# flyakon/DeepPhysiNet

Measured on AMD Instinct MI355X. Metric: collocation-points/sec (fwd+PDE-Jacobian+bwd), higher is better.
Workload: dtype bf16x2 (hi+lo split bf16 MFMA operands), fp32 accumulate

## Files before the change

deepphysinet_amd/csrc/dpn_encoder_chain.hip:

```cpp
#include <atomic>
#include <hip/hip_runtime.h>
#include <stdint.h>
#include <stdlib.h>

#include "../../include/dpn_hip.h"
#include "../../include/dpn_hip_experiments.h"

#define DEV __device__ __forceinline__

namespace {

typedef _Float16 f16x8 __attribute__((ext_vector_type(8)));
typedef float f32x4 __attribute__((ext_vector_type(4)));
typedef unsigned int u32;
typedef u32 u32x4 __attribute__((ext_vector_type(4)));

constexpr int kD = 256;
constexpr int kThreads = 512, kWaves = 8;
constexpr int kImgBytes = 256 * 1024;
#ifndef DPN_ENC_PF
#define DPN_ENC_PF 8
#endif
template <int NTT> constexpr int pf_of() { return NTT == 1 ? DPN_ENC_PF : 4; }
constexpr int kYS = 260;
constexpr int kXImg = 16384;
constexpr float kLoScale = 2048.0f, kLoInv = 1.0f / 2048.0f;

#ifdef DPN_ENC_TIMELINE
unsigned* g_enc_timeline = nullptr;
#define ENC_STAMP(I) do { if (a.tl && lane == 0) a.tl[((size_t)blockIdx.x * kWaves + wave) * 32 + (I)] = (unsigned)__builtin_readcyclecounter(); } while (0)
#define ENC_TL_ARG unsigned* tl;
#define ENC_TL_SET(A) (A).tl = g_enc_timeline
#else
#define ENC_STAMP(I) do { } while (0)
#define ENC_TL_ARG
#define ENC_TL_SET(A) do { } while (0)
#endif

DEV void barrier_lds() {
    __builtin_amdgcn_fence(__ATOMIC_RELEASE, "workgroup", "local");
    __builtin_amdgcn_s_barrier();
    __builtin_amdgcn_fence(__ATOMIC_ACQUIRE, "workgroup", "local");
}

template <int CTRL>
DEV float dpp(float v) { return __builtin_bit_cast(float, __builtin_amdgcn_update_dpp(0, __builtin_bit_cast(int, v), CTRL, 0xf, 0xf, false)); }
DEV float swz16(float v) { return __builtin_bit_cast(float, __builtin_amdgcn_ds_swizzle(__builtin_bit_cast(int, v), 0x401F)); }
DEV float half_sum(float v) {
    v += dpp<0xB1>(v);
    v += dpp<0x4E>(v);
    v += dpp<0x141>(v);
    v += dpp<0x140>(v);
    v += swz16(v);
    return v;
}
DEV float half_max(float v) {
    v = fmaxf(v, dpp<0xB1>(v));
    v = fmaxf(v, dpp<0x4E>(v));
    v = fmaxf(v, dpp<0x141>(v));
    v = fmaxf(v, dpp<0x140>(v));
    v = fmaxf(v, swz16(v));
    return v;
}

DEV float gelu_exact(float x) { return x * 0.5f * (1.0f + erff(x * 0.70710678118654752440f)); }
DEV float gelu_exact_grad(float x) {
    const float cdf = 0.5f * (1.0f + erff(x * 0.70710678118654752440f));
    const float pdf = expf(-0.5f * x * x) * 0.39894228040143267794f;
    return cdf + x * pdf;
}

DEV void split8(const float (&v)[8], u32x4& hi, u32x4& lo) {
    f16x8 h, l;
#pragma unroll
    for (int e = 0; e < 8; ++e) {
        const _Float16 a = (_Float16)v[e];
        h[e] = a;
        l[e] = (_Float16)((v[e] - (float)a) * kLoScale);
    }
    hi = __builtin_bit_cast(u32x4, h);
    lo = __builtin_bit_cast(u32x4, l);
}

DEV int xpos(int slot, int n) { return slot * 16 + (n ^ ((slot & 3) | ((slot & 4) ? 12 : 0))); }

struct RowLane {
    int tsel, slot, n16;
    DEV RowLane(int wave, int lane) : tsel(lane >> 5), slot(lane & 31), n16(2 * wave + (lane >> 5)) {}
};

DEV void row_to_ximg(const float (&v)[8], const float extra_max, const RowLane& rl, char* ximg_tile, float* rscale_tile) {
    float m = extra_max;
#pragma unroll
    for (int e = 0; e < 8; ++e) m = fmaxf(m, fabsf(v[e]));
    m = half_max(m);
    int eb = (__builtin_bit_cast(int, m) >> 23) & 0xff;
    eb = eb < 4 ? 4 : eb;
    const float sc = __builtin_bit_cast(float, (257 - eb) << 23);
    float s[8];
#pragma unroll
    for (int e = 0; e < 8; ++e) s[e] = v[e] * sc;
    u32x4 hi, lo;
    split8(s, hi, lo);
    char* p = ximg_tile + xpos(rl.slot, rl.n16) * 16;
    *reinterpret_cast<u32x4*>(p) = hi;
    *reinterpret_cast<u32x4*>(p + kXImg / 2) = lo;
    if (rl.slot == 0) rscale_tile[rl.n16] = __builtin_bit_cast(float, (eb - 3) << 23);
}
DEV float row_absmax(const float (&v)[8]) {
    float m = 0.f;
#pragma unroll
    for (int e = 0; e < 8; ++e) m = fmaxf(m, fabsf(v[e]));
    return m;
}

DEV void load8(float (&v)[8], const float* p, bool ok) {
    if (ok) {
        const float4 a = reinterpret_cast<const float4*>(p)[0], b = reinterpret_cast<const float4*>(p)[1];
        v[0] = a.x; v[1] = a.y; v[2] = a.z; v[3] = a.w; v[4] = b.x; v[5] = b.y; v[6] = b.z; v[7] = b.w;
    } else {
#pragma unroll
        for (int e = 0; e < 8; ++e) v[e] = 0.f;
    }
}
DEV void store8(float* p, const float (&v)[8], bool ok) {
    if (ok) {
        reinterpret_cast<float4*>(p)[0] = make_float4(v[0], v[1], v[2], v[3]);
        reinterpret_cast<float4*>(p)[1] = make_float4(v[4], v[5], v[6], v[7]);
    }
}
DEV void lds8(float (&v)[8], const float* p) {
    const f32x4 a = reinterpret_cast<const f32x4*>(p)[0], b = reinterpret_cast<const f32x4*>(p)[1];
    v[0] = a[0]; v[1] = a[1]; v[2] = a[2]; v[3] = a[3]; v[4] = b[0]; v[5] = b[1]; v[6] = b[2]; v[7] = b[3];
}

DEV void layer_norm8(const float (&v)[8], const float (&gam)[8], const float (&bet)[8], float (&xhat)[8], float (&y)[8], float& rstd) {
    float s = 0.f;
#pragma unroll
    for (int e = 0; e < 8; ++e) s += v[e];
    const float mean = half_sum(s) * (1.f / kD);
    float d[8], q = 0.f;
#pragma unroll
    for (int e = 0; e < 8; ++e) { d[e] = v[e] - mean; q = fmaf(d[e], d[e], q); }
    rstd = 1.0f / sqrtf(half_sum(q) * (1.f / kD) + 1e-5f);
#pragma unroll
    for (int e = 0; e < 8; ++e) { xhat[e] = d[e] * rstd; y[e] = fmaf(xhat[e], gam[e], bet[e]); }
}
DEV void layer_norm_bwd8(const float (&g)[8], const float (&xhat)[8], const float rstd, const float (&gam)[8], float (&gx)[8], float (&pg)[8],
                         float (&pb)[8]) {
    float t[8], s1 = 0.f, s2 = 0.f;
#pragma unroll
    for (int e = 0; e < 8; ++e) { t[e] = g[e] * gam[e]; s1 += t[e]; s2 = fmaf(t[e], xhat[e], s2); pg[e] = fmaf(g[e], xhat[e], pg[e]); pb[e] += g[e]; }
    const float m1 = half_sum(s1) * (1.f / kD), m2 = half_sum(s2) * (1.f / kD);
#pragma unroll
    for (int e = 0; e < 8; ++e) gx[e] = rstd * (t[e] - m1 - xhat[e] * m2);
}

struct WStream {
    __amdgpu_buffer_rsrc_t rs;
    int voff, tile_off;
    DEV void init(const void* wpack, int64_t bytes, int wave, int lane) {
        rs = __builtin_amdgcn_make_buffer_rsrc(const_cast<void*>(wpack), 0, (int)bytes, 0x00020000);
        voff = lane * 16;
        tile_off = wave * 2 * 16384;
    }
    DEV void load(u32x4 (&dst)[2][2], int img_off, int ks) const {
#pragma unroll
        for (int t = 0; t < 2; ++t)
#pragma unroll
            for (int p = 0; p < 2; ++p)
                dst[t][p] = __builtin_bit_cast(u32x4, __builtin_amdgcn_raw_buffer_load_b128(rs, voff + p * 1024, img_off + tile_off + t * 16384 + ks * 2048, 0));
    }
};
template <int PF> struct Ring { u32x4 a[PF][2][2]; };

DEV f32x4 mfma(u32x4 a, u32x4 b, f32x4 c) {
    return __builtin_amdgcn_mfma_f32_16x16x32_f16(__builtin_bit_cast(f16x8, a), __builtin_bit_cast(f16x8, b), c, 0, 0, 0);
}

template <int NTT>
struct Acc {
    f32x4 m[2][NTT], c[2][NTT];
    DEV void zero() {
#pragma unroll
        for (int t = 0; t < 2; ++t)
#pragma unroll
            for (int tt = 0; tt < NTT; ++tt) { m[t][tt] = (f32x4)0.f; c[t][tt] = (f32x4)0.f; }
    }
};

template <int NTT, bool HAS_NEXT>
DEV void gemm(const WStream& ws, Ring<pf_of<NTT>()>& R, const int cur_off, const int next_off, const char* xr0, const char* xr1, Acc<NTT>& acc) {
    u32x4 B[2][NTT][2];
    auto loadB = [&](const int ks, const int buf) __attribute__((always_inline)) {
        const char* base = ((ks & 1) ? xr1 : xr0) + ks * 1024;
#pragma unroll
        for (int tt = 0; tt < NTT; ++tt) {
            B[buf][tt][0] = *reinterpret_cast<const u32x4*>(base + tt * kXImg);
            B[buf][tt][1] = *reinterpret_cast<const u32x4*>(base + tt * kXImg + kXImg / 2);
        }
    };
    constexpr int kPF = pf_of<NTT>();
    loadB(0, 0);
#pragma unroll
    for (int ks = 0; ks < 8; ++ks) {
        if (ks + 1 < 8) loadB(ks + 1, (ks + 1) & 1);
        const int s = ks % kPF, b = ks & 1;
#pragma unroll
        for (int tt = 0; tt < NTT; ++tt) {
#pragma unroll
            for (int t = 0; t < 2; ++t) acc.m[t][tt] = mfma(R.a[s][t][0], B[b][tt][0], acc.m[t][tt]);
#pragma unroll
            for (int t = 0; t < 2; ++t) acc.c[t][tt] = mfma(R.a[s][t][0], B[b][tt][1], acc.c[t][tt]);
#pragma unroll
            for (int t = 0; t < 2; ++t) acc.c[t][tt] = mfma(R.a[s][t][1], B[b][tt][0], acc.c[t][tt]);
        }
        if (ks + kPF < 8) ws.load(R.a[s], cur_off, ks + kPF);
        else if (HAS_NEXT) ws.load(R.a[s], next_off, ks + kPF - 8);
    }
}

template <int NTT>
DEV void acc_to_staging(const Acc<NTT>& acc, float* Y, const float* rscale, int wave, int lane) {
    const int n = lane & 15, g = lane >> 4;
#pragma unroll
    for (int tt = 0; tt < NTT; ++tt) {
        const float rs = rscale[tt * 16 + n];
#pragma unroll
        for (int t = 0; t < 2; ++t) {
            f32x4 v;
#pragma unroll
            for (int j = 0; j < 4; ++j) v[j] = fmaf(acc.c[t][tt][j], kLoInv, acc.m[t][tt][j]) * rs;
            *reinterpret_cast<f32x4*>(Y + (tt * 16 + n) * kYS + wave * 32 + t * 16 + g * 4) = v;
        }
    }
}
template <int NTT>
DEV void acc_to_global(const Acc<NTT>& acc, float* out, const float* bias_lds, const float* rscale, int row0, int rows, int wave, int lane) {
    const int n = lane & 15, g = lane >> 4;
#pragma unroll
    for (int tt = 0; tt < NTT; ++tt) {
        const float rs = rscale[tt * 16 + n];
        const int row = row0 + tt * 16 + n;
#pragma unroll
        for (int t = 0; t < 2; ++t) {
            const int ch = wave * 32 + t * 16 + g * 4;
            f32x4 b = (f32x4)0.f;
            if (bias_lds) b = *reinterpret_cast<const f32x4*>(bias_lds + ch);
            f32x4 v;
#pragma unroll
            for (int j = 0; j < 4; ++j) v[j] = fmaf(acc.c[t][tt][j], kLoInv, acc.m[t][tt][j]) * rs + b[j];
            if (row < rows) *reinterpret_cast<f32x4*>(out + (int64_t)row * kD + ch) = v;
        }
    }
}

constexpr int kHelpers = 64;
DEV void l2_warm_helper(const void* wpack, const int (&img)[6], const int n_img, const int hb) {
    const int part = hb >> 3, t = threadIdx.x;
    float sum = 0.f;
    for (int i = t >> 8; i < n_img; i += 2) {
        const char* p = static_cast<const char*>(wpack) + img[i] + (part * 256 + (t & 255)) * 128;
        sum += *reinterpret_cast<const float*>(p);
    }
    asm volatile("" ::"v"(sum));
}

constexpr int kNVecF = 12;
enum { VF_BO = 0, VF_G1, VF_BE1, VF_BC1, VF_BC2, VF_G2, VF_BE2, VF_GF, VF_BEF, VF_BN0, VF_BN1, VF_BN2 };
struct FwdArgs {
    const void* wpack;
    int64_t wbytes;
    int img[6];
    int rows, n_main, n_img;
    const float *o, *x, *xin;
    const float* vec[kNVecF];
    float *x1, *xhat1, *rstd1, *pre, *act, *x2, *xhat2, *rstd2, *xf, *xhatf, *rstdf, *y0, *y1, *y2;
    const float *emb_parts, *emb_bias, *emb_pos, *emb_te, *emb_token;
    float* emb_out;
    int64_t emb_part_stride;
    int emb_n_parts, emb_n_tok;
    ENC_TL_ARG
};
template <int NTT>
struct Lds {
    static constexpr int kX = 0;
    static constexpr int kY = 3 * NTT * kXImg;
    static constexpr int kVec = kY + NTT * 16 * kYS * 4;
    static constexpr int kRs = kVec + kNVecF * 256 * 4;
    static constexpr int kRed = kRs + NTT * 16 * 4;
    static constexpr int kBytes = kRed + kWaves * 512 * 4;
};

constexpr int kEmbAhead = 9;
template <bool TAIL, int NEXT, int NTT>
__global__ __launch_bounds__(kThreads) void dpn_enc_fwd_kernel(FwdArgs a) {
    extern __shared__ __attribute__((aligned(16))) char smem[];
    char* ximg = smem + Lds<NTT>::kX;
    float* Y = reinterpret_cast<float*>(smem + Lds<NTT>::kY);
    float* vecs = reinterpret_cast<float*>(smem + Lds<NTT>::kVec);
    float* rscale = reinterpret_cast<float*>(smem + Lds<NTT>::kRs);
    const int tid = threadIdx.x, lane = tid & 63, wave = __builtin_amdgcn_readfirstlane(tid >> 6);
    if ((int)blockIdx.x >= a.n_main) { l2_warm_helper(a.wpack, a.img, a.n_img, blockIdx.x - a.n_main); return; }
    const int row0 = blockIdx.x * 16 * NTT;
    ENC_STAMP(0);
    const RowLane rl(wave, lane);
    const int n_r = lane & 15, g_r = lane >> 4;
    const char* xr0 = ximg + (g_r * 16 + (n_r ^ g_r)) * 16;
    const char* xr1 = ximg + (g_r * 16 + (n_r ^ g_r ^ 12)) * 16;
    float res[NTT][8], vin[NTT][8];
    bool ok[NTT];
#pragma unroll
    for (int tt = 0; tt < NTT; ++tt) {
        const int row = row0 + tt * 16 + rl.n16;
        ok[tt] = row < a.rows;
        if constexpr (!TAIL) {
            if (a.emb_parts) {
                const int c0 = rl.slot * 8;
                const bool tok = row < a.emb_n_tok;
                const int64_t po = ((int64_t)(tok ? 0 : row - a.emb_n_tok)) * kD + c0;
                float v[8];
                if (tok) load8(v, a.emb_token + (int64_t)row * kD + c0, ok[tt]);
                else load8(v, a.emb_parts + po, ok[tt]);
                if (!tok)
                    for (int p0 = 1; p0 < a.emb_n_parts; p0 += kEmbAhead) {
                        float t6[kEmbAhead][8];
#pragma unroll
                        for (int u = 0; u < kEmbAhead; ++u) load8(t6[u], a.emb_parts + (int64_t)min(p0 + u, a.emb_n_parts - 1) * a.emb_part_stride + po, ok[tt]);
#pragma unroll
                        for (int u = 0; u < kEmbAhead; ++u)
                            if (p0 + u < a.emb_n_parts) {
#pragma unroll
                                for (int e = 0; e < 8; ++e) v[e] += t6[u][e];
                            }
                    }
                float b8[8], p8[8], e8[8];
                load8(b8, a.emb_bias + c0, !tok && a.emb_bias != nullptr);
                load8(p8, a.emb_pos + (int64_t)row * kD + c0, ok[tt]);
                load8(e8, a.emb_te + c0, true);
#pragma unroll
                for (int e = 0; e < 8; ++e) vin[tt][e] = ok[tt] ? ((tok ? v[e] : v[e] + b8[e]) + p8[e]) + e8[e] : 0.f;
                store8(a.emb_out + (int64_t)row * kD + c0, vin[tt], ok[tt]);
                continue;
            }
        }
        load8(vin[tt], (TAIL ? a.o : a.xin) + (int64_t)row * kD + rl.slot * 8, ok[tt]);
        if constexpr (TAIL) load8(res[tt], a.x + (int64_t)row * kD + rl.slot * 8, ok[tt]);
    }
    constexpr int kVecLoads = (kNVecF * 64 + kThreads - 1) / kThreads;
    float4 pv[kVecLoads];
#pragma unroll
    for (int q = 0; q < kVecLoads; ++q) {
        const int i = tid + q * kThreads;
        const float* src = i < kNVecF * 64 ? a.vec[i >> 6] : nullptr;
        pv[q] = src ? reinterpret_cast<const float4*>(src)[i & 63] : make_float4(0.f, 0.f, 0.f, 0.f);
    }
    WStream ws;
    ws.init(a.wpack, a.wbytes, wave, lane);
    constexpr int kPF = pf_of<NTT>();
    Ring<kPF> R;
#pragma unroll
    for (int ks = 0; ks < kPF; ++ks) ws.load(R.a[ks], a.img[0], ks);
#pragma unroll
    for (int q = 0; q < kVecLoads; ++q) {
        const int i = tid + q * kThreads;
        if (i < kNVecF * 64) reinterpret_cast<float4*>(vecs)[i] = pv[q];
    }
#pragma unroll
    for (int tt = 0; tt < NTT; ++tt) row_to_ximg(vin[tt], 0.f, rl, ximg + tt * kXImg, rscale + tt * 16);
    ENC_STAMP(1);
    barrier_lds();
    ENC_STAMP(2);
    Acc<NTT> acc;
    constexpr int kFirstNext = TAIL ? 3 : 0;
    if constexpr (TAIL) {
        acc.zero();
        gemm<NTT, true>(ws, R, a.img[0], a.img[1], xr0, xr1, acc);
        ENC_STAMP(3);
        acc_to_staging<NTT>(acc, Y, rscale, wave, lane);
        barrier_lds();
        ENC_STAMP(4);
        float sa[NTT][8], sb[NTT][8], sr[NTT];
        {
            float gam[8], bet[8], bo[8];
            lds8(bo, vecs + VF_BO * 256 + rl.slot * 8); lds8(gam, vecs + VF_G1 * 256 + rl.slot * 8); lds8(bet, vecs + VF_BE1 * 256 + rl.slot * 8);
#pragma unroll
            for (int tt = 0; tt < NTT; ++tt) {
                float v[8];
                lds8(v, Y + (tt * 16 + rl.n16) * kYS + rl.slot * 8);
#pragma unroll
                for (int e = 0; e < 8; ++e) v[e] = res[tt][e] + (v[e] + bo[e]);
                layer_norm8(v, gam, bet, sb[tt], res[tt], sr[tt]);
                row_to_ximg(res[tt], 0.f, rl, ximg + tt * kXImg, rscale + tt * 16);
            }
        }
        ENC_STAMP(5);
        barrier_lds();
        ENC_STAMP(6);
#pragma unroll
        for (int tt = 0; tt < NTT; ++tt) {
            const int64_t off = (int64_t)(row0 + tt * 16 + rl.n16) * kD + rl.slot * 8;
            store8(a.x1 + off, res[tt], ok[tt]);
            store8(a.xhat1 + off, sb[tt], ok[tt]);
            if (ok[tt] && rl.slot == 0) a.rstd1[row0 + tt * 16 + rl.n16] = sr[tt];
        }
        acc.zero();
        gemm<NTT, true>(ws, R, a.img[1], a.img[2], xr0, xr1, acc);
        ENC_STAMP(7);
        acc_to_staging<NTT>(acc, Y, rscale, wave, lane);
        barrier_lds();
        ENC_STAMP(8);
        {
            float b1[8];
            lds8(b1, vecs + VF_BC1 * 256 + rl.slot * 8);
#pragma unroll
            for (int tt = 0; tt < NTT; ++tt) {
                lds8(sa[tt], Y + (tt * 16 + rl.n16) * kYS + rl.slot * 8);
#pragma unroll
                for (int e = 0; e < 8; ++e) { sa[tt][e] += b1[e]; sb[tt][e] = gelu_exact(sa[tt][e]); }
                row_to_ximg(sb[tt], 0.f, rl, ximg + tt * kXImg, rscale + tt * 16);
            }
        }
        ENC_STAMP(9);
        barrier_lds();
        ENC_STAMP(10);
#pragma unroll
        for (int tt = 0; tt < NTT; ++tt) {
            const int64_t off = (int64_t)(row0 + tt * 16 + rl.n16) * kD + rl.slot * 8;
            store8(a.pre + off, sa[tt], ok[tt]);
            store8(a.act + off, sb[tt], ok[tt]);
        }
        acc.zero();
        gemm<NTT, NEXT != 0>(ws, R, a.img[2], a.img[3], xr0, xr1, acc);
        ENC_STAMP(11);
        acc_to_staging<NTT>(acc, Y, rscale, wave, lane);
        barrier_lds();
        ENC_STAMP(12);
        float sc[NEXT == 2 ? NTT : 1][8], sd[NEXT == 2 ? NTT : 1][8], sq[NEXT == 2 ? NTT : 1];
        {
            float gam[8], bet[8], b2[8];
            lds8(b2, vecs + VF_BC2 * 256 + rl.slot * 8); lds8(gam, vecs + VF_G2 * 256 + rl.slot * 8); lds8(bet, vecs + VF_BE2 * 256 + rl.slot * 8);
#pragma unroll
            for (int tt = 0; tt < NTT; ++tt) {
                float v[8];
                lds8(v, Y + (tt * 16 + rl.n16) * kYS + rl.slot * 8);
#pragma unroll
                for (int e = 0; e < 8; ++e) v[e] = res[tt][e] + (v[e] + b2[e]);
                layer_norm8(v, gam, bet, sb[tt], sa[tt], sr[tt]);
                if constexpr (NEXT == 2) {
                    float gf[8], bf[8];
                    lds8(gf, vecs + VF_GF * 256 + rl.slot * 8); lds8(bf, vecs + VF_BEF * 256 + rl.slot * 8);
                    layer_norm8(sa[tt], gf, bf, sd[tt], sc[tt], sq[tt]);
                    row_to_ximg(sc[tt], 0.f, rl, ximg + tt * kXImg, rscale + tt * 16);
                } else if constexpr (NEXT == 1) {
                    row_to_ximg(sa[tt], 0.f, rl, ximg + tt * kXImg, rscale + tt * 16);
                }
            }
        }
        ENC_STAMP(13);
        if constexpr (NEXT != 0) barrier_lds();
        ENC_STAMP(14);
#pragma unroll
        for (int tt = 0; tt < NTT; ++tt) {
            const int64_t off = (int64_t)(row0 + tt * 16 + rl.n16) * kD + rl.slot * 8;
            store8(a.x2 + off, sa[tt], ok[tt]);
            store8(a.xhat2 + off, sb[tt], ok[tt]);
            if (ok[tt] && rl.slot == 0) a.rstd2[row0 + tt * 16 + rl.n16] = sr[tt];
            if constexpr (NEXT == 2) {
                store8(a.xf + off, sc[tt], ok[tt]);
                store8(a.xhatf + off, sd[tt], ok[tt]);
                if (ok[tt] && rl.slot == 0) a.rstdf[row0 + tt * 16 + rl.n16] = sq[tt];
            }
        }
    }
    if constexpr (NEXT == 1) {
        acc.zero();
        gemm<NTT, true>(ws, R, a.img[kFirstNext], a.img[kFirstNext + 1], xr0, xr1, acc);
        acc_to_global<NTT>(acc, a.y0, vecs + VF_BN0 * 256, rscale, row0, a.rows, wave, lane);
        ENC_STAMP(15);
        acc.zero();
        gemm<NTT, true>(ws, R, a.img[kFirstNext + 1], a.img[kFirstNext + 2], xr0, xr1, acc);
        acc_to_global<NTT>(acc, a.y1, vecs + VF_BN1 * 256, rscale, row0, a.rows, wave, lane);
        ENC_STAMP(16);
        acc.zero();
        gemm<NTT, false>(ws, R, a.img[kFirstNext + 2], 0, xr0, xr1, acc);
        acc_to_global<NTT>(acc, a.y2, vecs + VF_BN2 * 256, rscale, row0, a.rows, wave, lane);
        ENC_STAMP(17);
    } else if constexpr (NEXT == 2) {
        acc.zero();
        gemm<NTT, false>(ws, R, a.img[kFirstNext], 0, xr0, xr1, acc);
        acc_to_global<NTT>(acc, a.y0, vecs + VF_BN0 * 256, rscale, row0, a.rows, wave, lane);
    }
}

enum { VB_G2 = 0, VB_G1, VB_GF };
struct BwdArgs {
    const void* wpack;
    int64_t wbytes;
    int img[6];
    int rows, n_main, n_img;
    const float *res, *dq, *dk, *dv;
    const float *dmeta, *xhatf, *rstdf;
    const float* gin;
    const float *xhat2, *rstd2, *pre, *xhat1, *rstd1;
    const float* vec[3];
    float *gs2, *dpre, *gs1, *dout, *gx;
    float *partial_f, *partial2, *partial1;
    float* gx_head;
    int gx_head_rows;
    ENC_TL_ARG
};

DEV void partials_to_lds(float (&pg)[8], float (&pb)[8], float* red, int wave, int lane) {
#pragma unroll
    for (int e = 0; e < 8; ++e) { pg[e] += __shfl_xor(pg[e], 32); pb[e] += __shfl_xor(pb[e], 32); }
    if (lane < 32) {
        float* r = red + wave * 512 + lane * 8;
        reinterpret_cast<f32x4*>(r)[0] = (f32x4){pg[0], pg[1], pg[2], pg[3]};
        reinterpret_cast<f32x4*>(r)[1] = (f32x4){pg[4], pg[5], pg[6], pg[7]};
        reinterpret_cast<f32x4*>(r + 256)[0] = (f32x4){pb[0], pb[1], pb[2], pb[3]};
        reinterpret_cast<f32x4*>(r + 256)[1] = (f32x4){pb[4], pb[5], pb[6], pb[7]};
    }
}
DEV void partials_to_global(const float* red, float* partial, int tid) {
    float s = red[tid];
#pragma unroll
    for (int w = 1; w < kWaves; ++w) s += red[w * 512 + tid];
    partial[(int64_t)blockIdx.x * 512 + tid] = s;
}

template <int HEAD, bool BODY, int NTT>
__global__ __launch_bounds__(kThreads) void dpn_enc_bwd_kernel(BwdArgs a) {
    extern __shared__ __attribute__((aligned(16))) char smem[];
    char* ximg = smem + Lds<NTT>::kX;
    float* Y = reinterpret_cast<float*>(smem + Lds<NTT>::kY);
    float* vecs = reinterpret_cast<float*>(smem + Lds<NTT>::kVec);
    float* rscale = reinterpret_cast<float*>(smem + Lds<NTT>::kRs);
    float* red = reinterpret_cast<float*>(smem + Lds<NTT>::kRed);
    const int tid = threadIdx.x, lane = tid & 63, wave = __builtin_amdgcn_readfirstlane(tid >> 6);
    if ((int)blockIdx.x >= a.n_main) { l2_warm_helper(a.wpack, a.img, a.n_img, blockIdx.x - a.n_main); return; }
    const int row0 = blockIdx.x * 16 * NTT;
    ENC_STAMP(0);
    const RowLane rl(wave, lane);
    const int n_r = lane & 15, g_r = lane >> 4;
    const char* xr0 = ximg + (g_r * 16 + (n_r ^ g_r)) * 16;
    const char* xr1 = ximg + (g_r * 16 + (n_r ^ g_r ^ 12)) * 16;
    bool ok[NTT];
    int64_t off[NTT];
#pragma unroll
    for (int tt = 0; tt < NTT; ++tt) {
        const int row = row0 + tt * 16 + rl.n16;
        ok[tt] = row < a.rows;
        off[tt] = (int64_t)row * kD + rl.slot * 8;
    }
    float hq[HEAD == 1 ? NTT : 1][8], hk[HEAD == 1 ? NTT : 1][8], hv[NTT][8], g[NTT][8];
    float xhf[HEAD == 2 ? NTT : 1][8], rsf[HEAD == 2 ? NTT : 1];
#pragma unroll
    for (int tt = 0; tt < NTT; ++tt) {
        if constexpr (HEAD == 1) {
            load8(hq[tt], a.dq + off[tt], ok[tt]); load8(hk[tt], a.dk + off[tt], ok[tt]); load8(hv[tt], a.dv + off[tt], ok[tt]);
        } else if constexpr (HEAD == 2) {
            load8(hv[tt], a.dmeta + off[tt], ok[tt]);
        } else {
            load8(g[tt], a.gin + off[tt], ok[tt]);
        }
    }
    float4 pv = make_float4(0.f, 0.f, 0.f, 0.f);
    if (tid < 3 * 64) {
        const float* src = a.vec[tid >> 6];
        if (src) pv = reinterpret_cast<const float4*>(src)[tid & 63];
    }
    WStream ws;
    ws.init(a.wpack, a.wbytes, wave, lane);
    constexpr int kPF = pf_of<NTT>();
    Ring<kPF> R;
#pragma unroll
    for (int ks = 0; ks < kPF; ++ks) ws.load(R.a[ks], a.img[0], ks);
    float xh2[BODY ? NTT : 1][8], prv[BODY ? NTT : 1][8], xh1[BODY ? NTT : 1][8], rs2[BODY ? NTT : 1], rs1[BODY ? NTT : 1];
#pragma unroll
    for (int tt = 0; tt < NTT; ++tt) {
        if constexpr (HEAD == 1) load8(g[tt], a.res + off[tt], ok[tt]);
        if constexpr (HEAD == 2) {
            load8(xhf[tt], a.xhatf + off[tt], ok[tt]);
            rsf[tt] = ok[tt] ? a.rstdf[row0 + tt * 16 + rl.n16] : 0.f;
        }
        if constexpr (BODY) {
            load8(xh2[tt], a.xhat2 + off[tt], ok[tt]);
            load8(prv[tt], a.pre + off[tt], ok[tt]);
            load8(xh1[tt], a.xhat1 + off[tt], ok[tt]);
            rs2[tt] = ok[tt] ? a.rstd2[row0 + tt * 16 + rl.n16] : 0.f;
            rs1[tt] = ok[tt] ? a.rstd1[row0 + tt * 16 + rl.n16] : 0.f;
        }
    }
    if (tid < 3 * 64) reinterpret_cast<float4*>(vecs)[tid] = pv;
    Acc<NTT> acc;
    constexpr int kHeadImgs = HEAD == 1 ? 3 : HEAD == 2 ? 1 : 0;
    if constexpr (HEAD == 1) {
#pragma unroll
        for (int tt = 0; tt < NTT; ++tt) {
            const float m = fmaxf(row_absmax(hq[tt]), fmaxf(row_absmax(hk[tt]), row_absmax(hv[tt])));
            row_to_ximg(hq[tt], m, rl, ximg + tt * kXImg, rscale + tt * 16);
            row_to_ximg(hk[tt], m, rl, ximg + (NTT + tt) * kXImg, rscale + tt * 16);
            row_to_ximg(hv[tt], m, rl, ximg + (2 * NTT + tt) * kXImg, rscale + tt * 16);
        }
        ENC_STAMP(1);
        barrier_lds();
        ENC_STAMP(2);
        acc.zero();
        gemm<NTT, true>(ws, R, a.img[0], a.img[1], xr0, xr1, acc);
        gemm<NTT, true>(ws, R, a.img[1], a.img[2], xr0 + NTT * kXImg, xr1 + NTT * kXImg, acc);
        gemm<NTT, BODY>(ws, R, a.img[2], a.img[3], xr0 + 2 * NTT * kXImg, xr1 + 2 * NTT * kXImg, acc);
        ENC_STAMP(3);
        acc_to_staging<NTT>(acc, Y, rscale, wave, lane);
        barrier_lds();
        ENC_STAMP(4);
#pragma unroll
        for (int tt = 0; tt < NTT; ++tt) {
            float v[8];
            lds8(v, Y + (tt * 16 + rl.n16) * kYS + rl.slot * 8);
#pragma unroll
            for (int e = 0; e < 8; ++e) g[tt][e] += v[e];
        }
    } else if constexpr (HEAD == 2) {
#pragma unroll
// ... 589 lines not shown
        a.p[i] = WgProblem{q.A, q.B, q.C, q.asum, q.bias, q.M, q.N, q.K, q.ldc, q.a_sm, q.a_sk, q.b_sn, q.b_sk, off};
        const int64_t per = (int64_t)q.M * q.N + (q.asum ? q.M : 0);
        off += (int64_t)slices * per;
        per_max = per_max > per ? per_max : per;
        const int tx = (q.N + kWgTile - 1) / kWgTile, ty = (q.M + kWgTile - 1) / kWgTile;
        if ((int64_t)tx * ty > (1 << 20) || tiles + (int64_t)tx * ty * slices > (1 << 30)) return -1;
        a.start[i] = (int)tiles;
        a.tx[i] = tx; a.per_slice[i] = tx * ty; a.inv_tx[i] = 1.0f / (float)tx;
        tiles += (int64_t)tx * ty * slices;
        max_k = max_k > q.K ? max_k : q.K;
    }
    for (int i = n; i <= kWgMaxProblems; ++i) a.start[i] = (int)tiles;
    a.n_tiles = (int)tiles;
    a.rows_per_slice = ((max_k + slices - 1) / slices + 31) / 32 * 32;
    for (int i = 0; i < n_jobs; ++i) {
        if (!jobs[i].partial || !jobs[i].out_a || !jobs[i].out_b || jobs[i].n_blocks <= 0) return -1;
        a.job[i] = WgJob{jobs[i].partial, jobs[i].out_a, jobs[i].out_b, jobs[i].n_blocks, 0};
    }
    hipStream_t s = reinterpret_cast<hipStream_t>(stream);
    hipLaunchKernelGGL(dpn_wgrad16_kernel, dim3((unsigned)tiles + n_jobs), dim3(64 * kWgWaves), 0, s, a);
    if (slices > 1 && n > 0 && reduce)
        hipLaunchKernelGGL(dpn_wgrad16_reduce_kernel, dim3((unsigned)((per_max + 255) / 256), n), dim3(256), 0, s, a);
    return (int)hipGetLastError();
}

static int64_t gemm16_partial_floats(int n, const DpnGemm16Problem* problems, int slices) {
    if (n <= 0 || !problems || slices <= 1) return 0;
    int64_t tot = 0;
    for (int i = 0; i < n; ++i) tot += (int64_t)slices * ((int64_t)problems[i].M * problems[i].N + (problems[i].asum ? problems[i].M : 0));
    return tot;
}
static int wgrad_as_gemm16(int n, const DpnWgradProblem* problems, DpnGemm16Problem* out) {
    for (int i = 0; i < n; ++i) {
        const DpnWgradProblem& q = problems[i];
        if (!q.G || !q.X || !q.dW || q.M <= 0 || q.N <= 0 || q.rows <= 0 || q.ldg < q.M || q.ldx < q.N || q.ldw < q.N) return -1;
        out[i] = DpnGemm16Problem{q.G, q.X, q.dW, q.db, nullptr, q.M, q.N, q.rows, q.ldw, 1, q.ldg, 1, q.ldx};
    }
    return 0;
}

int64_t dpn_wgrad16_partial_floats(int n, const DpnWgradProblem* problems, int slices) {
    if (n <= 0 || n > kWgMaxProblems || !problems || slices <= 1) return 0;
    DpnGemm16Problem g[kWgMaxProblems];
    if (wgrad_as_gemm16(n, problems, g)) return 0;
    return gemm16_partial_floats(n, g, slices);
}

int dpn_wgrad16(int n, const DpnWgradProblem* problems, int n_jobs, const DpnColsumJob* jobs, int slices, float* partials, void* stream) {
    if (n < 0 || n > kWgMaxProblems || (n && !problems)) return -1;
    DpnGemm16Problem g[kWgMaxProblems];
    if (wgrad_as_gemm16(n, problems, g)) return -1;
    return gemm16_launch(n, g, n_jobs, jobs, slices, partials, 1, stream);
}

int dpn_attn16_fwd(const float* q, const float* k, const float* v, int L, int batch, float* out, float* P, void* stream) {
    if (!q || !k || !v || !out || !P || L <= 0 || L > kALmax || batch <= 0 || batch > 32767) return -1;
    Attn16Args a{q, k, v, out, P, L, 1.0f / sqrtf(32.0f)};
    hipLaunchKernelGGL(dpn_attn16_fwd_kernel, dim3((L + 15) / 16, 8, batch), dim3(256), 0, reinterpret_cast<hipStream_t>(stream), a);
    return (int)hipGetLastError();
}

int dpn_enc_prep(const DpnEncPrep* p, void* stream) {
    if (!p || p->n_mats < 0 || p->n_mats > DPN_ENC_MAX_MATS || (p->n_mats && (!p->weights || !p->packed))) return -1;
    if ((p->x != nullptr) != (p->xu != nullptr) || (p->x && (p->T <= 0 || p->C <= 0 || p->batch <= 0))) return -1;
    if (p->h && (p->batch <= 0 || !p->freqs_a || !p->out_a || p->n_a <= 0 || p->n_b < 0 || (p->n_b > 0 && (!p->freqs_b || !p->out_b)))) return -1;
    PrepArgs a{};
    for (int i = 0; i < p->n_mats; ++i) {
        if (!p->weights[i]) return -1;
        a.pack.W[i] = p->weights[i];
    }
    a.pack.n = p->n_mats; a.pack.out = static_cast<char*>(p->packed); a.pack.status = p->status_dev;
    a.pack_blocks = p->n_mats * 64;
    a.x = p->x; a.T = p->T; a.C = p->C; a.xu = p->xu;
    a.col_total = p->x ? (int64_t)p->batch * p->T * p->C * 3 : 0;
    a.col_blocks = (int)((a.col_total + 255) / 256);
    a.h = p->h; a.batch = p->batch; a.fa = p->freqs_a; a.na = p->n_a; a.oa = p->out_a; a.fb = p->freqs_b; a.nb = p->h ? p->n_b : 0; a.ob = p->out_b;
    const int pe_blocks = p->h ? (p->batch * (p->n_a + a.nb) + 255) / 256 : 0;
    const int blocks = a.pack_blocks + a.col_blocks + pe_blocks;
    if (blocks <= 0) return -1;
    hipLaunchKernelGGL(dpn_enc_prep_kernel, dim3(blocks), dim3(256), 0, reinterpret_cast<hipStream_t>(stream), a);
    return (int)hipGetLastError();
}

int dpn_enc_fwd(const DpnEncFwd* p, void* stream) {
    if (!p || !p->wpack || p->rows <= 0 || p->n_mats <= 0 || p->n_mats > DPN_ENC_MAX_MATS || p->next < 0 || p->next > 2) return -1;
    if (!p->tail && p->next != 1) return -1;
    const bool wide = p->row_tiles == 2;
    if (p->row_tiles != 1 && p->row_tiles != 2) return -1;
    FwdArgs a{};
    a.wpack = p->wpack; a.wbytes = dpn_enc_pack_bytes(p->n_mats); a.rows = p->rows;
    auto mat_ok = [&](int m) { return m >= 0 && m < p->n_mats; };
    int ni = 0;
    if (p->tail) {
        if (!mat_ok(p->m_o) || !mat_ok(p->m_c1) || !mat_ok(p->m_c2)) return -1;
        if (!p->o || !p->x || !p->bo || !p->g1 || !p->be1 || !p->bc1 || !p->bc2 || !p->g2 || !p->be2) return -1;
        if (!p->x1 || !p->xhat1 || !p->rstd1 || !p->pre || !p->act || !p->x2 || !p->xhat2 || !p->rstd2) return -1;
        a.img[ni++] = img_off(p->m_o, 0); a.img[ni++] = img_off(p->m_c1, 0); a.img[ni++] = img_off(p->m_c2, 0);
    } else if (p->emb_parts) {
        if (!p->emb_pos || !p->emb_te || !p->emb_out || p->emb_n_parts < 1 || p->emb_n_tok < 0 || (p->emb_n_tok > 0 && !p->emb_token) || p->emb_part_stride < 0) return -1;
        a.emb_parts = p->emb_parts; a.emb_bias = p->emb_bias; a.emb_pos = p->emb_pos; a.emb_te = p->emb_te; a.emb_token = p->emb_token; a.emb_out = p->emb_out;
        a.emb_part_stride = p->emb_part_stride; a.emb_n_parts = p->emb_n_parts; a.emb_n_tok = p->emb_n_tok;
    } else if (!p->xin) return -1;
    if (p->next == 1) {
        if (!mat_ok(p->m_n0) || !mat_ok(p->m_n1) || !mat_ok(p->m_n2) || !p->y0 || !p->y1 || !p->y2) return -1;
        a.img[ni++] = img_off(p->m_n0, 0); a.img[ni++] = img_off(p->m_n1, 0); a.img[ni++] = img_off(p->m_n2, 0);
    } else if (p->next == 2) {
        if (!mat_ok(p->m_n0) || !p->y0 || !p->gf || !p->bef || !p->xf || !p->xhatf || !p->rstdf) return -1;
        a.img[ni++] = img_off(p->m_n0, 0);
    }
    a.o = p->o; a.x = p->x; a.xin = p->xin;
    const float* vec[kNVecF] = {p->bo, p->g1, p->be1, p->bc1, p->bc2, p->g2, p->be2, p->gf, p->bef, p->bn0, p->bn1, p->bn2};
    for (int i = 0; i < kNVecF; ++i) a.vec[i] = vec[i];
    a.x1 = p->x1; a.xhat1 = p->xhat1; a.rstd1 = p->rstd1; a.pre = p->pre; a.act = p->act; a.x2 = p->x2; a.xhat2 = p->xhat2; a.rstd2 = p->rstd2;
    a.xf = p->xf; a.xhatf = p->xhatf; a.rstdf = p->rstdf; a.y0 = p->y0; a.y1 = p->y1; a.y2 = p->y2;
    ENC_TL_SET(a);
    hipStream_t s = reinterpret_cast<hipStream_t>(stream);
    const int rpw = wide ? 32 : 16;
    a.n_main = (p->rows + rpw - 1) / rpw; a.n_img = ni;
    const dim3 grid(a.n_main + (a.n_main <= 64 ? kHelpers : 0)), block(kThreads);
    static std::atomic<unsigned long long> done{0};
    unsigned long long dev_bit;
#define DPN_ENC_FWD_CASES(X) X(true, 0) X(true, 1) X(true, 2) X(false, 1)
    if (first_use_on_device(done, dev_bit)) {
#define X(T, N) if (set_lds(dpn_enc_fwd_kernel<T, N, 1>, Lds<1>::kBytes) || set_lds(dpn_enc_fwd_kernel<T, N, 2>, Lds<2>::kBytes)) return -2;
        DPN_ENC_FWD_CASES(X)
#undef X
        done.fetch_or(dev_bit, std::memory_order_release);
    }
#define X(T, N) if ((p->tail != 0) == T && p->next == N) { \
        if (wide) hipLaunchKernelGGL((dpn_enc_fwd_kernel<T, N, 2>), grid, block, Lds<2>::kBytes, s, a); \
        else hipLaunchKernelGGL((dpn_enc_fwd_kernel<T, N, 1>), grid, block, Lds<1>::kBytes, s, a); }
    DPN_ENC_FWD_CASES(X)
#undef X
    return (int)hipGetLastError();
}

int dpn_enc_bwd(const DpnEncBwd* p, void* stream) {
    if (!p || p->rows <= 0 || p->head < 0 || p->head > 2 || (p->row_tiles != 1 && p->row_tiles != 2)) return -1;
    if (p->head == 0 && !p->body) return -1;
    if (!p->wpack || p->n_mats <= 0 || p->n_mats > DPN_ENC_MAX_MATS) return -1;
    const bool wide = p->row_tiles == 2;
    BwdArgs a{};
    a.wpack = p->wpack; a.wbytes = dpn_enc_pack_bytes(p->n_mats); a.rows = p->rows;
    auto mat_ok = [&](int m) { return m >= 0 && m < p->n_mats; };
    int ni = 0;
    if (p->head == 1) {
        if (!mat_ok(p->m_h0) || !mat_ok(p->m_h1) || !mat_ok(p->m_h2) || !p->res || !p->dq || !p->dk || !p->dv) return -1;
        a.img[ni++] = img_off(p->m_h0, 1); a.img[ni++] = img_off(p->m_h1, 1); a.img[ni++] = img_off(p->m_h2, 1);
    } else if (p->head == 2) {
        if (!mat_ok(p->m_h0) || !p->dmeta || !p->xhatf || !p->rstdf || !p->gf || !p->partial_f) return -1;
        a.img[ni++] = img_off(p->m_h0, 1);
    } else if (!p->gin) return -1;
    if (p->body) {
        if (!mat_ok(p->m_c2) || !mat_ok(p->m_c1) || !mat_ok(p->m_o)) return -1;
        if (!p->xhat2 || !p->rstd2 || !p->pre || !p->xhat1 || !p->rstd1 || !p->g2 || !p->g1) return -1;
        if (!p->gs2 || !p->dpre || !p->gs1 || !p->dout || !p->partial2 || !p->partial1) return -1;
        a.img[ni++] = img_off(p->m_c2, 1); a.img[ni++] = img_off(p->m_c1, 1); a.img[ni++] = img_off(p->m_o, 1);
    } else if (!p->gx) return -1;
    a.res = p->res; a.dq = p->dq; a.dk = p->dk; a.dv = p->dv; a.dmeta = p->dmeta; a.xhatf = p->xhatf; a.rstdf = p->rstdf; a.gin = p->gin;
    a.xhat2 = p->xhat2; a.rstd2 = p->rstd2; a.pre = p->pre; a.xhat1 = p->xhat1; a.rstd1 = p->rstd1;
    a.vec[VB_G2] = p->g2; a.vec[VB_G1] = p->g1; a.vec[VB_GF] = p->gf;
    a.gs2 = p->gs2; a.dpre = p->dpre; a.gs1 = p->gs1; a.dout = p->dout; a.gx = p->gx;
    a.gx_head = p->gx_head; a.gx_head_rows = (p->gx_head && !p->body) ? p->gx_head_rows : 0;
    a.partial_f = p->partial_f; a.partial2 = p->partial2; a.partial1 = p->partial1;
    ENC_TL_SET(a);
    hipStream_t s = reinterpret_cast<hipStream_t>(stream);
    const int rpw = wide ? 32 : 16;
    a.n_main = (p->rows + rpw - 1) / rpw; a.n_img = ni;
    const dim3 grid(a.n_main + (a.n_main <= 64 && ni > 0 ? kHelpers : 0)), block(kThreads);
    static std::atomic<unsigned long long> done{0};
    unsigned long long dev_bit;
#define DPN_ENC_BWD_CASES(X) X(0, true) X(1, true) X(2, true) X(1, false)
    if (first_use_on_device(done, dev_bit)) {
#define X(H, B) if (set_lds(dpn_enc_bwd_kernel<H, B, 1>, Lds<1>::kBytes) || set_lds(dpn_enc_bwd_kernel<H, B, 2>, Lds<2>::kBytes)) return -2;
        DPN_ENC_BWD_CASES(X)
#undef X
        done.fetch_or(dev_bit, std::memory_order_release);
    }
#define X(H, B) if (p->head == H && (p->body != 0) == B) { \
        if (wide) hipLaunchKernelGGL((dpn_enc_bwd_kernel<H, B, 2>), grid, block, Lds<2>::kBytes, s, a); \
        else hipLaunchKernelGGL((dpn_enc_bwd_kernel<H, B, 1>), grid, block, Lds<1>::kBytes, s, a); }
    DPN_ENC_BWD_CASES(X)
#undef X
    return (int)hipGetLastError();
}

}
```

Before: 34.70 million.

## Replicate small-batch encoder workgroups across q/k/v projections to fill idle CUs

When the row count is small enough that the grid leaves compute units idle, the forward encoder kernel launches three replicas per row block, each computing one of the q/k/v output projections, with only replica 0 writing the shared intermediates. The backward head-only path gets a new kernel that splits the 256 output channels across two workgroups per row block, each accumulating across the three projection GEMMs for its half. This spreads the serialized final GEMMs across more CUs to shorten the critical path, at the cost of redundant recomputation of the earlier encoder layers in each replica and extra weight traffic.

```diff
diff --git a/deepphysinet_amd/csrc/dpn_encoder_chain.hip b/deepphysinet_amd/csrc/dpn_encoder_chain.hip
--- a/deepphysinet_amd/csrc/dpn_encoder_chain.hip
+++ b/deepphysinet_amd/csrc/dpn_encoder_chain.hip
@@ -28,7 +28,7 @@
 
 #ifdef DPN_ENC_TIMELINE
 unsigned* g_enc_timeline = nullptr;
-#define ENC_STAMP(I) do { if (a.tl && lane == 0) a.tl[((size_t)blockIdx.x * kWaves + wave) * 32 + (I)] = (unsigned)__builtin_readcyclecounter(); } while (0)
+#define ENC_STAMP(I) do { if (a.tl && lane == 0) a.tl[((size_t)tl_block * kWaves + wave) * 32 + (I)] = (unsigned)__builtin_readcyclecounter(); } while (0)
 #define ENC_TL_ARG unsigned* tl;
 #define ENC_TL_SET(A) (A).tl = g_enc_timeline
 #else
@@ -164,33 +164,34 @@
         voff = lane * 16;
         tile_off = wave * 2 * 16384;
     }
-    DEV void load(u32x4 (&dst)[2][2], int img_off, int ks) const {
-#pragma unroll
-        for (int t = 0; t < 2; ++t)
+    template <int NT>
+    DEV void load(u32x4 (&dst)[NT][2], int img_off, int ks) const {
+#pragma unroll
+        for (int t = 0; t < NT; ++t)
 #pragma unroll
             for (int p = 0; p < 2; ++p)
                 dst[t][p] = __builtin_bit_cast(u32x4, __builtin_amdgcn_raw_buffer_load_b128(rs, voff + p * 1024, img_off + tile_off + t * 16384 + ks * 2048, 0));
     }
 };
-template <int PF> struct Ring { u32x4 a[PF][2][2]; };
+template <int PF, int NT = 2> struct Ring { u32x4 a[PF][NT][2]; };
 
 DEV f32x4 mfma(u32x4 a, u32x4 b, f32x4 c) {
     return __builtin_amdgcn_mfma_f32_16x16x32_f16(__builtin_bit_cast(f16x8, a), __builtin_bit_cast(f16x8, b), c, 0, 0, 0);
 }
 
-template <int NTT>
+template <int NTT, int NT = 2>
 struct Acc {
-    f32x4 m[2][NTT], c[2][NTT];
+    f32x4 m[NT][NTT], c[NT][NTT];
     DEV void zero() {
 #pragma unroll
-        for (int t = 0; t < 2; ++t)
+        for (int t = 0; t < NT; ++t)
 #pragma unroll
             for (int tt = 0; tt < NTT; ++tt) { m[t][tt] = (f32x4)0.f; c[t][tt] = (f32x4)0.f; }
     }
 };
 
-template <int NTT, bool HAS_NEXT>
-DEV void gemm(const WStream& ws, Ring<pf_of<NTT>()>& R, const int cur_off, const int next_off, const char* xr0, const char* xr1, Acc<NTT>& acc) {
+template <int NTT, bool HAS_NEXT, int NT = 2>
+DEV void gemm(const WStream& ws, Ring<pf_of<NTT>(), NT>& R, const int cur_off, const int next_off, const char* xr0, const char* xr1, Acc<NTT, NT>& acc) {
     u32x4 B[2][NTT][2];
     auto loadB = [&](const int ks, const int buf) __attribute__((always_inline)) {
         const char* base = ((ks & 1) ? xr1 : xr0) + ks * 1024;
@@ -209,29 +210,29 @@
 #pragma unroll
         for (int tt = 0; tt < NTT; ++tt) {
 #pragma unroll
-            for (int t = 0; t < 2; ++t) acc.m[t][tt] = mfma(R.a[s][t][0], B[b][tt][0], acc.m[t][tt]);
-#pragma unroll
-            for (int t = 0; t < 2; ++t) acc.c[t][tt] = mfma(R.a[s][t][0], B[b][tt][1], acc.c[t][tt]);
-#pragma unroll
-            for (int t = 0; t < 2; ++t) acc.c[t][tt] = mfma(R.a[s][t][1], B[b][tt][0], acc.c[t][tt]);
+            for (int t = 0; t < NT; ++t) acc.m[t][tt] = mfma(R.a[s][t][0], B[b][tt][0], acc.m[t][tt]);
+#pragma unroll
+            for (int t = 0; t < NT; ++t) acc.c[t][tt] = mfma(R.a[s][t][0], B[b][tt][1], acc.c[t][tt]);
+#pragma unroll
+            for (int t = 0; t < NT; ++t) acc.c[t][tt] = mfma(R.a[s][t][1], B[b][tt][0], acc.c[t][tt]);
         }
         if (ks + kPF < 8) ws.load(R.a[s], cur_off, ks + kPF);
         else if (HAS_NEXT) ws.load(R.a[s], next_off, ks + kPF - 8);
     }
 }
 
-template <int NTT>
-DEV void acc_to_staging(const Acc<NTT>& acc, float* Y, const float* rscale, int wave, int lane) {
+template <int NTT, int NT = 2>
+DEV void acc_to_staging(const Acc<NTT, NT>& acc, float* Y, const float* rscale, int wave, int lane, const int first_tile = 0) {
     const int n = lane & 15, g = lane >> 4;
 #pragma unroll
     for (int tt = 0; tt < NTT; ++tt) {
         const float rs = rscale[tt * 16 + n];
 #pragma unroll
-        for (int t = 0; t < 2; ++t) {
+        for (int t = 0; t < NT; ++t) {
             f32x4 v;
 #pragma unroll
             for (int j = 0; j < 4; ++j) v[j] = fmaf(acc.c[t][tt][j], kLoInv, acc.m[t][tt][j]) * rs;
-            *reinterpret_cast<f32x4*>(Y + (tt * 16 + n) * kYS + wave * 32 + t * 16 + g * 4) = v;
+            *reinterpret_cast<f32x4*>(Y + (tt * 16 + n) * kYS + wave * 32 + (NT == 2 ? t : first_tile) * 16 + g * 4) = v;
         }
     }
 }
@@ -256,6 +257,8 @@
 }
 
 constexpr int kHelpers = 64;
+constexpr int kHelperMaxMain = 64;
+constexpr int kCUs = 256;
 DEV void l2_warm_helper(const void* wpack, const int (&img)[6], const int n_img, const int hb) {
     const int part = hb >> 3, t = threadIdx.x;
     float sum = 0.f;
@@ -293,16 +296,30 @@
 };
 
 constexpr int kEmbAhead = 9;
-template <bool TAIL, int NEXT, int NTT>
+#ifndef DPN_ENC_REP_ROW_MAJOR
+#define DPN_ENC_REP_ROW_MAJOR 0
+#endif
+template <bool TAIL, int NEXT, int NTT, int REP = 1>
 __global__ __launch_bounds__(kThreads) void dpn_enc_fwd_kernel(FwdArgs a) {
+    static_assert(REP == 1 || (REP == 3 && NEXT == 1 && NTT == 1), "replicas: one per q / k / v projection, 16-row workgroups only");
     extern __shared__ __attribute__((aligned(16))) char smem[];
     char* ximg = smem + Lds<NTT>::kX;
     float* Y = reinterpret_cast<float*>(smem + Lds<NTT>::kY);
     float* vecs = reinterpret_cast<float*>(smem + Lds<NTT>::kVec);
     float* rscale = reinterpret_cast<float*>(smem + Lds<NTT>::kRs);
     const int tid = threadIdx.x, lane = tid & 63, wave = __builtin_amdgcn_readfirstlane(tid >> 6);
-    if ((int)blockIdx.x >= a.n_main) { l2_warm_helper(a.wpack, a.img, a.n_img, blockIdx.x - a.n_main); return; }
-    const int row0 = blockIdx.x * 16 * NTT;
+    if ((int)blockIdx.x >= a.n_main * REP) { l2_warm_helper(a.wpack, a.img, a.n_img, blockIdx.x - a.n_main * REP); return; }
+    int rb = blockIdx.x, rep = 0;
+    if constexpr (REP == 3) {
+        if (DPN_ENC_REP_ROW_MAJOR) { rb = (int)blockIdx.x / 3; rep = (int)blockIdx.x - 3 * rb; }
+        else { rep = ((int)blockIdx.x >= a.n_main) + ((int)blockIdx.x >= 2 * a.n_main); rb = (int)blockIdx.x - rep * a.n_main; }
+    }
+    const bool keeper = REP == 1 || rep == 0;
+    constexpr int kFirstNext = TAIL ? 3 : 0;
+    const int rep_img = REP == 1 ? 0 : rep == 0 ? a.img[kFirstNext] : rep == 1 ? a.img[kFirstNext + 1] : a.img[kFirstNext + 2];
+    float* const rep_y = REP == 1 ? nullptr : rep == 0 ? a.y0 : rep == 1 ? a.y1 : a.y2;
+    const int row0 = rb * 16 * NTT;
+    [[maybe_unused]] const int tl_block = rep * a.n_main + rb;
     ENC_STAMP(0);
     const RowLane rl(wave, lane);
     const int n_r = lane & 15, g_r = lane >> 4;
@@ -340,7 +357,7 @@
                 load8(e8, a.emb_te + c0, true);
 #pragma unroll
                 for (int e = 0; e < 8; ++e) vin[tt][e] = ok[tt] ? ((tok ? v[e] : v[e] + b8[e]) + p8[e]) + e8[e] : 0.f;
-                store8(a.emb_out + (int64_t)row * kD + c0, vin[tt], ok[tt]);
+                store8(a.emb_out + (int64_t)row * kD + c0, vin[tt], ok[tt] && keeper);
                 continue;
             }
         }
@@ -360,7 +377,7 @@
     constexpr int kPF = pf_of<NTT>();
     Ring<kPF> R;
 #pragma unroll
-    for (int ks = 0; ks < kPF; ++ks) ws.load(R.a[ks], a.img[0], ks);
+    for (int ks = 0; ks < kPF; ++ks) ws.load(R.a[ks], (!TAIL && REP == 3) ? rep_img : a.img[0], ks);
 #pragma unroll
     for (int q = 0; q < kVecLoads; ++q) {
         const int i = tid + q * kThreads;
@@ -372,8 +389,10 @@
     barrier_lds();
     ENC_STAMP(2);
     Acc<NTT> acc;
-    constexpr int kFirstNext = TAIL ? 3 : 0;
     if constexpr (TAIL) {
+        bool okst[NTT];
+#pragma unroll
+        for (int tt = 0; tt < NTT; ++tt) okst[tt] = ok[tt] && keeper;
         acc.zero();
         gemm<NTT, true>(ws, R, a.img[0], a.img[1], xr0, xr1, acc);
         ENC_STAMP(3);
@@ -400,9 +419,9 @@
 #pragma unroll
         for (int tt = 0; tt < NTT; ++tt) {
             const int64_t off = (int64_t)(row0 + tt * 16 + rl.n16) * kD + rl.slot * 8;
-            store8(a.x1 + off, res[tt], ok[tt]);
-            store8(a.xhat1 + off, sb[tt], ok[tt]);
-            if (ok[tt] && rl.slot == 0) a.rstd1[row0 + tt * 16 + rl.n16] = sr[tt];
+            store8(a.x1 + off, res[tt], okst[tt]);
+            store8(a.xhat1 + off, sb[tt], okst[tt]);
+            if (okst[tt] && rl.slot == 0) a.rstd1[row0 + tt * 16 + rl.n16] = sr[tt];
         }
         acc.zero();
         gemm<NTT, true>(ws, R, a.img[1], a.img[2], xr0, xr1, acc);
@@ -427,11 +446,11 @@
 #pragma unroll
         for (int tt = 0; tt < NTT; ++tt) {
             const int64_t off = (int64_t)(row0 + tt * 16 + rl.n16) * kD + rl.slot * 8;
-            store8(a.pre + off, sa[tt], ok[tt]);
-            store8(a.act + off, sb[tt], ok[tt]);
+            store8(a.pre + off, sa[tt], okst[tt]);
+            store8(a.act + off, sb[tt], okst[tt]);
         }
         acc.zero();
-        gemm<NTT, NEXT != 0>(ws, R, a.img[2], a.img[3], xr0, xr1, acc);
+        gemm<NTT, NEXT != 0>(ws, R, a.img[2], REP == 3 ? rep_img : a.img[3], xr0, xr1, acc);
         ENC_STAMP(11);
         acc_to_staging<NTT>(acc, Y, rscale, wave, lane);
         barrier_lds();
@@ -463,9 +482,9 @@
 #pragma unroll
         for (int tt = 0; tt < NTT; ++tt) {
             const int64_t off = (int64_t)(row0 + tt * 16 + rl.n16) * kD + rl.slot * 8;
-            store8(a.x2 + off, sa[tt], ok[tt]);
-            store8(a.xhat2 + off, sb[tt], ok[tt]);
-            if (ok[tt] && rl.slot == 0) a.rstd2[row0 + tt * 16 + rl.n16] = sr[tt];
+            store8(a.x2 + off, sa[tt], okst[tt]);
+            store8(a.xhat2 + off, sb[tt], okst[tt]);
+            if (okst[tt] && rl.slot == 0) a.rstd2[row0 + tt * 16 + rl.n16] = sr[tt];
             if constexpr (NEXT == 2) {
                 store8(a.xf + off, sc[tt], ok[tt]);
                 store8(a.xhatf + off, sd[tt], ok[tt]);
@@ -473,7 +492,12 @@
             }
         }
     }
-    if constexpr (NEXT == 1) {
+    if constexpr (NEXT == 1 && REP == 3) {
+        acc.zero();
+        gemm<NTT, false>(ws, R, rep_img, 0, xr0, xr1, acc);
+        acc_to_global<NTT>(acc, rep_y, vecs + (VF_BN0 + rep) * 256, rscale, row0, a.rows, wave, lane);
+        ENC_STAMP(17);
+    } else if constexpr (NEXT == 1) {
         acc.zero();
         gemm<NTT, true>(ws, R, a.img[kFirstNext], a.img[kFirstNext + 1], xr0, xr1, acc);
         acc_to_global<NTT>(acc, a.y0, vecs + VF_BN0 * 256, rscale, row0, a.rows, wave, lane);
@@ -529,6 +553,61 @@
     partial[(int64_t)blockIdx.x * 512 + tid] = s;
 }
 
+__global__ __launch_bounds__(kThreads) void dpn_enc_bwd_qkv2_kernel(BwdArgs a) {
+    extern __shared__ __attribute__((aligned(16))) char smem[];
+    char* ximg = smem + Lds<1>::kX;
+    float* Y = reinterpret_cast<float*>(smem + Lds<1>::kY);
+    float* rscale = reinterpret_cast<float*>(smem + Lds<1>::kRs);
+    const int tid = threadIdx.x, lane = tid & 63, wave = __builtin_amdgcn_readfirstlane(tid >> 6);
+    if ((int)blockIdx.x >= 2 * a.n_main) { l2_warm_helper(a.wpack, a.img, a.n_img, blockIdx.x - 2 * a.n_main); return; }
+    const int rep = (int)blockIdx.x >= a.n_main, rb = (int)blockIdx.x - rep * a.n_main;
+    const int row0 = rb * 16;
+    [[maybe_unused]] const int tl_block = blockIdx.x;
+    ENC_STAMP(0);
+    const RowLane rl(wave, lane);
+    const int n_r = lane & 15, g_r = lane >> 4;
+    const char* xr0 = ximg + (g_r * 16 + (n_r ^ g_r)) * 16;
+    const char* xr1 = ximg + (g_r * 16 + (n_r ^ g_r ^ 12)) * 16;
+    const int row = row0 + rl.n16;
+    const bool ok = row < a.rows;
+    const bool mine = ok && ((rl.slot >> 1) & 1) == rep;
+    const int64_t off = (int64_t)row * kD + rl.slot * 8;
+    float hq[8], hk[8], hv[8], g[8];
+    load8(hq, a.dq + off, ok); load8(hk, a.dk + off, ok); load8(hv, a.dv + off, ok);
+    WStream ws;
+    ws.init(a.wpack, a.wbytes, wave, lane);
+    ws.tile_off += rep * 16384;
+    constexpr int kPF = pf_of<1>();
+    Ring<kPF, 1> R;
+#pragma unroll
+    for (int ks = 0; ks < kPF; ++ks) ws.load(R.a[ks], a.img[0], ks);
+    load8(g, a.res + off, mine);
+    const float m = fmaxf(row_absmax(hq), fmaxf(row_absmax(hk), row_absmax(hv)));
+    row_to_ximg(hq, m, rl, ximg, rscale);
+    row_to_ximg(hk, m, rl, ximg + kXImg, rscale);
+    row_to_ximg(hv, m, rl, ximg + 2 * kXImg, rscale);
+    ENC_STAMP(1);
+    barrier_lds();
+    ENC_STAMP(2);
+    Acc<1, 1> acc;
+    acc.zero();
+    gemm<1, true, 1>(ws, R, a.img[0], a.img[1], xr0, xr1, acc);
+    gemm<1, true, 1>(ws, R, a.img[1], a.img[2], xr0 + kXImg, xr1 + kXImg, acc);
+    gemm<1, false, 1>(ws, R, a.img[2], 0, xr0 + 2 * kXImg, xr1 + 2 * kXImg, acc);
+    ENC_STAMP(3);
+    acc_to_staging<1, 1>(acc, Y, rscale, wave, lane, rep);
+    barrier_lds();
+    ENC_STAMP(4);
+    if (mine) {
+        float v[8];
+        lds8(v, Y + rl.n16 * kYS + rl.slot * 8);
+#pragma unroll
+        for (int e = 0; e < 8; ++e) g[e] += v[e];
+        store8(a.gx + off, g, true);
+        if (row < a.gx_head_rows) store8(a.gx_head + off, g, true);
+    }
+}
+
 template <int HEAD, bool BODY, int NTT>
 __global__ __launch_bounds__(kThreads) void dpn_enc_bwd_kernel(BwdArgs a) {
     extern __shared__ __attribute__((aligned(16))) char smem[];
@@ -540,6 +619,7 @@
     const int tid = threadIdx.x, lane = tid & 63, wave = __builtin_amdgcn_readfirstlane(tid >> 6);
     if ((int)blockIdx.x >= a.n_main) { l2_warm_helper(a.wpack, a.img, a.n_img, blockIdx.x - a.n_main); return; }
     const int row0 = blockIdx.x * 16 * NTT;
+    [[maybe_unused]] const int tl_block = blockIdx.x;
     ENC_STAMP(0);
     const RowLane rl(wave, lane);
     const int n_r = lane & 15, g_r = lane >> 4;
@@ -1295,6 +1375,17 @@
     return (int)hipGetLastError();
 }
 
+int dpn_enc_fwd_replicas(int rows, int row_tiles, int tail, int next) {
+    (void)tail;
+    if (rows <= 0 || row_tiles != 1 || next != 1) return 1;
+    const int n_main = (rows + 15) / 16;
+#ifdef DPN_ENC_REP_MAX_MAIN
+    return n_main <= DPN_ENC_REP_MAX_MAIN ? 3 : 1;
+#else
+    return n_main * 3 + (n_main <= kHelperMaxMain ? kHelpers : 0) <= kCUs ? 3 : 1;
+#endif
+}
+
 int dpn_enc_fwd(const DpnEncFwd* p, void* stream) {
     if (!p || !p->wpack || p->rows <= 0 || p->n_mats <= 0 || p->n_mats > DPN_ENC_MAX_MATS || p->next < 0 || p->next > 2) return -1;
     if (!p->tail && p->next != 1) return -1;
@@ -1330,7 +1421,8 @@
     hipStream_t s = reinterpret_cast<hipStream_t>(stream);
     const int rpw = wide ? 32 : 16;
     a.n_main = (p->rows + rpw - 1) / rpw; a.n_img = ni;
-    const dim3 grid(a.n_main + (a.n_main <= 64 ? kHelpers : 0)), block(kThreads);
+    const int reps = dpn_enc_fwd_replicas(p->rows, p->row_tiles, p->tail, p->next);
+    const dim3 grid(a.n_main * reps + (a.n_main <= kHelperMaxMain ? kHelpers : 0)), block(kThreads);
     static std::atomic<unsigned long long> done{0};
     unsigned long long dev_bit;
 #define DPN_ENC_FWD_CASES(X) X(true, 0) X(true, 1) X(true, 2) X(false, 1)
@@ -1338,7 +1430,13 @@
 #define X(T, N) if (set_lds(dpn_enc_fwd_kernel<T, N, 1>, Lds<1>::kBytes) || set_lds(dpn_enc_fwd_kernel<T, N, 2>, Lds<2>::kBytes)) return -2;
         DPN_ENC_FWD_CASES(X)
 #undef X
+        if (set_lds(dpn_enc_fwd_kernel<true, 1, 1, 3>, Lds<1>::kBytes) || set_lds(dpn_enc_fwd_kernel<false, 1, 1, 3>, Lds<1>::kBytes)) return -2;
         done.fetch_or(dev_bit, std::memory_order_release);
+    }
+    if (reps == 3) {
+        if (p->tail) hipLaunchKernelGGL((dpn_enc_fwd_kernel<true, 1, 1, 3>), grid, block, Lds<1>::kBytes, s, a);
+        else hipLaunchKernelGGL((dpn_enc_fwd_kernel<false, 1, 1, 3>), grid, block, Lds<1>::kBytes, s, a);
+        return (int)hipGetLastError();
     }
 #define X(T, N) if ((p->tail != 0) == T && p->next == N) { \
         if (wide) hipLaunchKernelGGL((dpn_enc_fwd_kernel<T, N, 2>), grid, block, Lds<2>::kBytes, s, a); \
@@ -1346,6 +1444,16 @@
     DPN_ENC_FWD_CASES(X)
 #undef X
     return (int)hipGetLastError();
+}
+
+int dpn_enc_bwd_replicas(int rows, int row_tiles, int head, int body) {
+    if (rows <= 0 || row_tiles != 1 || head != 1 || body != 0) return 1;
+    const int n_main = (rows + 15) / 16;
+#ifdef DPN_ENC_BWD_REP_MAX_MAIN
+    return n_main <= DPN_ENC_BWD_REP_MAX_MAIN ? 2 : 1;
+#else
+    return n_main * 2 + (n_main <= kHelperMaxMain ? kHelpers : 0) <= kCUs ? 2 : 1;
+#endif
 }
 
 int dpn_enc_bwd(const DpnEncBwd* p, void* stream) {
@@ -1380,7 +1488,8 @@
     hipStream_t s = reinterpret_cast<hipStream_t>(stream);
     const int rpw = wide ? 32 : 16;
     a.n_main = (p->rows + rpw - 1) / rpw; a.n_img = ni;
-    const dim3 grid(a.n_main + (a.n_main <= 64 && ni > 0 ? kHelpers : 0)), block(kThreads);
+    const int reps = dpn_enc_bwd_replicas(p->rows, p->row_tiles, p->head, p->body);
+    const dim3 grid(a.n_main * reps + (a.n_main <= kHelperMaxMain && ni > 0 ? kHelpers : 0)), block(kThreads);
     static std::atomic<unsigned long long> done{0};
     unsigned long long dev_bit;
 #define DPN_ENC_BWD_CASES(X) X(0, true) X(1, true) X(2, true) X(1, false)
@@ -1388,7 +1497,12 @@
 #define X(H, B) if (set_lds(dpn_enc_bwd_kernel<H, B, 1>, Lds<1>::kBytes) || set_lds(dpn_enc_bwd_kernel<H, B, 2>, Lds<2>::kBytes)) return -2;
         DPN_ENC_BWD_CASES(X)
 #undef X
+        if (set_lds(dpn_enc_bwd_qkv2_kernel, Lds<1>::kBytes)) return -2;
         done.fetch_or(dev_bit, std::memory_order_release);
+    }
+    if (reps == 2) {
+        hipLaunchKernelGGL(dpn_enc_bwd_qkv2_kernel, grid, block, Lds<1>::kBytes, s, a);
+        return (int)hipGetLastError();
     }
 #define X(H, B) if (p->head == H && (p->body != 0) == B) { \
         if (wide) hipLaunchKernelGGL((dpn_enc_bwd_kernel<H, B, 2>), grid, block, Lds<2>::kBytes, s, a); \
```

Result: faster. 35.34 million (median of 6 runs) (+1.8%).
